# facebookresearch/PoseDiffusion

Measured on AMD Instinct MI355X. Metric: sequences/sec (20-frame, GGS on), higher is better.
Workload: dtype f32 (GGS, attention, LayerNorm, DDPM update, every accumulation); the encoder GEMMs multiply fp16 hi + lo operand pairs (22 bits, static power-of-two scales) with fp32 accumulation -- `exact_mode` is the same pipe with them on the exact-fp32 matrix instruction

## Files before the change

### posediffusion_amd/csrc/pd_denoiser.hip

```cpp
#include "pd_denoiser_dev.h"
#include "pd_gemm_stream.h"
#include "pd_gemm_split.h"
#include "pd_qkv_attn.h"
#ifndef PD_STRIP_RT3
#define PD_STRIP_RT3 1
#endif
#ifndef PD_STRIP_RT1
#define PD_STRIP_RT1 0
#endif
#ifndef PD_STRIP_RT3_FF1
#define PD_STRIP_RT3_FF1 0
#endif
#ifndef PD_STRIP_K64
#define PD_STRIP_K64 true
#endif

#include <algorithm>
#include <math.h>
#include <stdlib.h>
#include <string.h>

__global__ __launch_bounds__(256) void pd_embed_rows_kernel(const float *__restrict__ x, int n_frames, int M, float *__restrict__ out) {
    const int row = blockIdx.x * 4 + (threadIdx.x >> 6), lane = threadIdx.x & 63;
    if (row >= M) return;
    float4 *dst = (float4 *)(out + (size_t)row * KFIRST_D);
    float xv[9];
#pragma unroll
    for (int d = 0; d < 9; ++d) xv[d] = x[(size_t)row * 9 + d];
    if (lane < 45) {
        float o[4];
#pragma unroll
        for (int e = 0; e < 4; ++e) {
            const int idx = 4 * lane + e, s = idx / 90, rem = idx - s * 90, d = rem / 10, kk = rem - d * 10;
            float xd = xv[0];
#pragma unroll
            for (int q = 1; q < 9; ++q) xd = (d == q) ? xv[q] : xd;
            const float a = xd * (float)(1 << kk);
// ... 656 lines not shown
            pd_set_error("pd_engine_create: a LayerNorm weight pointer is NULL");
            return PD_ERR_INVALID_ARG;
        }
        PD_TRY(m.fold_bias(&L.qkv_b, s.in_proj_w, s.norm1_b, s.in_proj_b, 3 * DM, DM));
        PD_TRY(m.copy(&L.out_b, s.out_proj_b, DM));
        PD_TRY(m.fold_bias(&L.ff1_b, s.linear1_w, s.norm2_b, s.linear1_b, DFF, DM));
        PD_TRY(m.copy(&L.ff2_b, s.linear2_b, DM));
        PD_TRY(m.rowmajor(&L.qkv_wf, s.in_proj_w, 3 * DM, DM, s.norm1_w));
        PD_TRY(m.rowmajor(&L.out_wf, s.out_proj_w, DM, DM, nullptr));
        PD_TRY(m.rowmajor(&L.ff1_wf, s.linear1_w, DFF, DM, s.norm2_w));
        PD_TRY(m.rowmajor(&L.ff2_wf, s.linear2_w, DM, DFF, nullptr));
    }
    PD_TRY(m.copy(&d->last0_b, w->last0_b, HID));
    PD_TRY(m.copy(&d->last_ln_w, w->last_ln_w, HID));
    PD_TRY(m.copy(&d->last_ln_b, w->last_ln_b, HID));
    PD_TRY(m.copy(&d->last3_w, w->last3_w, 9 * HID));
    PD_TRY(m.copy(&d->last3_b, w->last3_b, 9));
    const size_t rows = (size_t)d->m_cap;
    PD_TRY(m.alloc(&d->h, rows * DM));
    PD_TRY(m.alloc(&d->qkv, rows * 3 * DM));
    PD_TRY(m.alloc(&d->ctx, rows * DM));
    PD_TRY(m.alloc(&d->ff, rows * DFF));
    PD_TRY(m.alloc(&d->hid, rows * HID));
    if (rows >= PD_STREAM_MIN_ROWS) PD_TRY(m.alloc(&d->hn, rows * DM));
    if (d->hn) {
        PD_TRY(m.alloc(&d->emb, rows * KFIRST_D));
        PD_TRY(m.alloc(&d->zproj, rows * DM));
        PD_TRY(m.alloc(&d->first_df, (size_t)DM * KFIRST_D));
        PD_TRY(m.alloc(&d->first_zf, (size_t)DM * ZD));
        hipLaunchKernelGGL(pd_first_rowmajor_kernel, dim3((DM * KFIRST_D + 255) / 256), dim3(256), 0, 0, w->first_w, d->first_df, PD_FIRST_D, KFIRST_D);
        hipLaunchKernelGGL(pd_first_rowmajor_kernel, dim3((DM * ZD + 255) / 256), dim3(256), 0, 0, w->first_w, d->first_zf, PD_FIRST_Z, ZD);
        PD_HIP_CHECK(hipGetLastError());
        PD_TRY(m.alloc(&d->ttab, (size_t)w->timesteps * DM));
        hipLaunchKernelGGL(pd_first_ttab_kernel, dim3(w->timesteps), dim3(DM), 0, 0, w->first_w, d->t_table, d->ttab);
        PD_HIP_CHECK(hipGetLastError());
    }
    PD_TRY(m.rowmajor(&d->last0_wf, w->last0_w, HID, DM, nullptr));
    PD_TRY(pd_set_lds(pd_gemm_kernel<KFIRST_PAD, 2, 0, 32>, 32 * (KFIRST_PAD + 4) * 4));
    PD_TRY(pd_set_lds(pd_gemm_kernel<KFIRST_PAD, 2, 0, 16>, 32 * (KFIRST_PAD + 4) * 4));
    PD_TRY(pd_set_lds(pd_gemm_kernel<DM, 1, 0, 32>, 32 * (DM + 4) * 4));
    PD_TRY(pd_set_lds(pd_gemm_kernel<DM, 1, 0, 16>, 32 * (DM + 4) * 4));
    PD_TRY(pd_set_lds(pd_gemm_kernel<DM, 1, 1, 32>, 32 * (DM + 4) * 4));
    PD_TRY(pd_set_lds(pd_gemm_kernel<DM, 1, 1, 16>, 32 * (DM + 4) * 4));
    PD_TRY(pd_set_lds(pd_gemm_kernel<DM, 0, 2, 32>, 32 * (DM + 4) * 4));
    PD_TRY(pd_set_lds(pd_gemm_kernel<DM, 0, 2, 16>, 32 * (DM + 4) * 4));
    PD_TRY(pd_set_lds(pd_gemm_kernel<DFF, 0, 2, 32>, 32 * (DFF + 4) * 4));
    PD_TRY(pd_set_lds(pd_gemm_kernel<DFF, 0, 2, 16>, 32 * (DFF + 4) * 4));
// ... 135 lines not shown
                     eng->max_B, eng->max_N, d->timesteps);
        return PD_ERR_INVALID_ARG;
    }
    if (!z_prepared) {
        int rc = pd_denoiser_prepare(eng, z, B, N, s);
        if (rc) return rc;
    }
    const int M = B * N, MT = (M + 31) / 32;
    GemmArgs g;
    memset(&g, 0, sizeof(g));
    g.M = M;
    const bool streamed = M >= PD_STREAM_MIN_ROWS && d->hn;
    if (streamed) {
        hipLaunchKernelGGL(pd_embed_rows_kernel, dim3((M + 3) / 4), dim3(256), 0, s, x, N, M, d->emb);
        pd_gemm_dma<4>(d->emb, KFIRST_D, d->first_df, KFIRST_D, d->ttab + (size_t)t * DM, d->h, M, DM, s, nullptr, d->zproj);
    } else {
        g.bias = d->first_b; g.C = d->h; g.Nout = DM;
        g.x = x; g.z = z; g.temb = d->t_table + (size_t)t * 128; g.n_frames = N;
        launch_gemm<KFIRST_PAD, 2, 0>(g, d->first_wp, MT, eng->gemm_wide_min_tiles, s);
    }
    for (int l = 0; l < d->num_layers; ++l) {
        const PdLayerDev &L = d->layers[l];
        if (streamed && eng->den_split == 2 && d->split_h_ready) {
            static const int strip = pd_dev_knob("PD_DEN_STRIP", 15);
            hipLaunchKernelGGL((pd_ln_rows_kernel<DM, 2>), dim3((M + 3) / 4), dim3(256), 0, s, d->h, d->hn, M, 1e-5f, 512.0f);
            static const int attn_mma = pd_dev_knob("PD_DEN_ATTN_MMA", 1);
            const int qa_wgs = ((B + pd_qkv_attn_group(N > 32 ? 1 : N) - 1) / pd_qkv_attn_group(N > 32 ? 1 : N)) * NH, cus = eng->num_cus > 0 ? eng->num_cus : 256;
            const bool qa_fills = 4 * qa_wgs >= 3 * ((qa_wgs + cus - 1) / cus) * cus;
            if (N <= 32 && eng->den_fused_attn == 1 ? qa_fills : (N <= 32 && eng->den_fused_attn == 2)) {
                pd_qkv_attn((const unsigned *)d->hn, L.qkv_wh, L.qkv_b, (unsigned *)d->ctx, B, N, L.qkv_cs, L.ctx_scale, s);
            } else {
                if (strip & 1) pd_gemm_strip<0, 2, true, 1, PD_STRIP_K64>((const unsigned *)d->hn, DM, L.qkv_wh, DM, L.qkv_b, d->qkv, M, 3 * DM, s, L.qkv_cs);
                else pd_gemm_split<0, 1, 2, true>((const unsigned *)d->hn, DM, L.qkv_wh, DM, L.qkv_b, d->qkv, M, 3 * DM, s, L.qkv_cs);
                if (N <= 32 && attn_mma) hipLaunchKernelGGL(pd_attn_mma_kernel<2>, dim3(B * NH), dim3(256), attn_mma_lds(N), s, d->qkv, d->ctx, N, L.ctx_scale);
                else hipLaunchKernelGGL(pd_attn_seq_kernel<2>, dim3(B * NH), dim3(256), attn_seq_lds(N), s, d->qkv, d->ctx, N, L.ctx_scale);
            }
            const bool rt3 = PD_STRIP_RT3 && (((M + 63) / 64) * (DM / 128)) > cus && (((M + 95) / 96) * (DM / 128)) <= cus;
#if PD_STRIP_RT1
            if ((strip & 2) && rt3) pd_gemm_strip<2, 1, true, 1, PD_STRIP_K64>((const unsigned *)d->ctx, DM, L.out_wh, DM, L.out_b, d->h, M, DM, s, L.out_cs);
            else
#endif
            if ((strip & 2) && rt3) pd_gemm_strip<2, 3, true, 1, PD_STRIP_K64>((const unsigned *)d->ctx, DM, L.out_wh, DM, L.out_b, d->h, M, DM, s, L.out_cs);
            else if (strip & 2) pd_gemm_strip<2, 2, true, 1, PD_STRIP_K64>((const unsigned *)d->ctx, DM, L.out_wh, DM, L.out_b, d->h, M, DM, s, L.out_cs);
            else pd_gemm_split<2, 1, 1, true>((const unsigned *)d->ctx, DM, L.out_wh, DM, L.out_b, d->h, M, DM, s, L.out_cs);
            hipLaunchKernelGGL((pd_ln_rows_kernel<DM, 2>), dim3((M + 3) / 4), dim3(256), 0, s, d->h, d->hn, M, 1e-5f, 512.0f);
#if PD_STRIP_RT1 == 2
            if ((strip & 4) && rt3) pd_gemm_strip<4, 1, true, 1, PD_STRIP_K64>((const unsigned *)d->hn, DM, L.ff1_wh, DM, L.ff1_b, d->ff, M, DFF, s, L.ff1_cs, L.ff_scale);
            else
#endif
            if ((strip & 4) && PD_STRIP_RT3_FF1 && rt3) pd_gemm_strip<4, 3, true, 1, PD_STRIP_K64>((const unsigned *)d->hn, DM, L.ff1_wh, DM, L.ff1_b, d->ff, M, DFF, s, L.ff1_cs, L.ff_scale);
            else if (strip & 4) pd_gemm_strip<4, 2, true, 1, PD_STRIP_K64>((const unsigned *)d->hn, DM, L.ff1_wh, DM, L.ff1_b, d->ff, M, DFF, s, L.ff1_cs, L.ff_scale);
            else pd_gemm_split<4, 1, 2, true>((const unsigned *)d->hn, DM, L.ff1_wh, DM, L.ff1_b, d->ff, M, DFF, s, L.ff1_cs, L.ff_scale);
#if PD_STRIP_RT1
            if ((strip & 8) && rt3) pd_gemm_strip<2, 1, true, 1, PD_STRIP_K64>((const unsigned *)d->ff, DFF, L.ff2_wh, DFF, L.ff2_b, d->h, M, DM, s, L.ff2_cs);
            else
#endif
            if ((strip & 8) && rt3) pd_gemm_strip<2, 3, true, 1, PD_STRIP_K64>((const unsigned *)d->ff, DFF, L.ff2_wh, DFF, L.ff2_b, d->h, M, DM, s, L.ff2_cs);
            else if (strip & 8) pd_gemm_strip<2, 2, true, 1, PD_STRIP_K64>((const unsigned *)d->ff, DFF, L.ff2_wh, DFF, L.ff2_b, d->h, M, DM, s, L.ff2_cs);
            else pd_gemm_split<2, 1, 1, true>((const unsigned *)d->ff, DFF, L.ff2_wh, DFF, L.ff2_b, d->h, M, DM, s, L.ff2_cs);
            continue;
        }
        if (streamed && eng->den_split == 1 && d->split_ready) {
            hipLaunchKernelGGL((pd_ln_rows_kernel<DM, 1>), dim3((M + 3) / 4), dim3(256), 0, s, d->h, d->hn, M, 1e-5f, 1.0f);
            pd_gemm_split<0, 1, 2>((const unsigned *)d->hn, DM, L.qkv_ws, DM, L.qkv_b, d->qkv, M, 3 * DM, s);
            hipLaunchKernelGGL(pd_attn_seq_kernel<1>, dim3(B * NH), dim3(256), attn_seq_lds(N), s, d->qkv, d->ctx, N, 1.0f);
            pd_gemm_split<2, 1, 1>((const unsigned *)d->ctx, DM, L.out_ws, DM, L.out_b, d->h, M, DM, s);
            hipLaunchKernelGGL((pd_ln_rows_kernel<DM, 1>), dim3((M + 3) / 4), dim3(256), 0, s, d->h, d->hn, M, 1e-5f, 1.0f);
            pd_gemm_split<4, 1, 2>((const unsigned *)d->hn, DM, L.ff1_ws, DM, L.ff1_b, d->ff, M, DFF, s);
            pd_gemm_split<2, 1, 1>((const unsigned *)d->ff, DFF, L.ff2_ws, DFF, L.ff2_b, d->h, M, DM, s);
            continue;
        }
        if (streamed) {
            float2 *stats = (float2 *)d->hn;
            hipLaunchKernelGGL(pd_ln_stats_kernel<DM>, dim3((M + 3) / 4), dim3(256), 0, s, d->h, stats, M, 1e-5f);
            pd_gemm_dma<0, true>(d->h, DM, L.qkv_wf, DM, L.qkv_b, d->qkv, M, 3 * DM, s, stats);
            hipLaunchKernelGGL(pd_attn_seq_kernel<0>, dim3(B * NH), dim3(256), attn_seq_lds(N), s, d->qkv, d->ctx, N, 1.0f);
            pd_gemm_dma<2>(d->ctx, DM, L.out_wf, DM, L.out_b, d->h, M, DM, s);
            hipLaunchKernelGGL(pd_ln_stats_kernel<DM>, dim3((M + 3) / 4), dim3(256), 0, s, d->h, stats, M, 1e-5f);
            pd_gemm_dma<1, true>(d->h, DM, L.ff1_wf, DM, L.ff1_b, d->ff, M, DFF, s, stats);
            pd_gemm_dma<2>(d->ff, DFF, L.ff2_wf, DFF, L.ff2_b, d->h, M, DM, s);
            continue;
        }
// ... 101 lines not shown
```

### posediffusion_amd/csrc/pd_denoiser_dev.h

```cpp
#pragma once
#include "pd_weight_prep.h"

#include <vector>

typedef float f32x16 __attribute__((ext_vector_type(16)));
typedef float f32x4 __attribute__((ext_vector_type(4)));

#define DM 512
#define NH 4
#define DH 128
#define DFF 1024
#define ZD 384
#define KFIRST 702
#define KFIRST_PAD 704
__host__ __device__ inline int pd_first_col_all(int kp) {
    if (kp < 384) return 317 + kp;
    if (kp < 512) return 189 + (kp - 384);
    if (kp < 692) return kp - 512;
    if (kp < 701) return 180 + (kp - 692);
    return kp;
}
#define PD_FIRST_D 1
#define PD_FIRST_Z 2
#define PD_FIRST_T 3
// ... 8 lines not shown

struct PdLayerDev {
    float *qkv_wp[2], *qkv_b;
    float *out_wp[2], *out_b;
    float *ff1_wp[2], *ff1_b;
    float *ff2_wp[2], *ff2_b;
    float *qkv_wf, *out_wf, *ff1_wf, *ff2_wf;
    unsigned *qkv_ws, *out_ws, *ff1_ws, *ff2_ws;
    unsigned *qkv_wh, *out_wh, *ff1_wh, *ff2_wh;
    float qkv_cs, out_cs, ff1_cs, ff2_cs, ctx_scale, ff_scale;
};

struct PdDenoiserDev {
    int num_layers = 0, timesteps = 0, m_cap = 0;
    float *t_table = nullptr;
    float *first_wp[2] = {nullptr, nullptr}, *first_b = nullptr;
    float *ttab = nullptr;
    float *zproj = nullptr;
    PdLayerDev layers[PD_MAX_LAYERS];
    float *last0_wp[2] = {nullptr, nullptr}, *last0_b = nullptr, *last_ln_w = nullptr, *last_ln_b = nullptr;
    float *last3_w = nullptr, *last3_b = nullptr;
    float *h = nullptr, *qkv = nullptr, *ctx = nullptr, *ff = nullptr, *hid = nullptr;
    float *hn = nullptr;
    float *emb = nullptr, *first_df = nullptr, *first_zf = nullptr, *last0_wf = nullptr;
    bool split_ready = false;
    bool split_h_ready = false;
    bool non_finite = false;
    PdDevAllocs mem{"pd_engine_create"};
};

template <int CTRL>
__device__ __forceinline__ float pd_dpp_add(float v) {
    return v + __int_as_float(__builtin_amdgcn_update_dpp(0, __float_as_int(v), CTRL, 0xf, 0xf, false));
}
__device__ __forceinline__ float pd_sum8(float v) {
    v = pd_dpp_add<0xB1>(v);
    v = pd_dpp_add<0x4E>(v);
    return pd_dpp_add<0x141>(v);
}

__device__ __forceinline__ float pd_wave_max(float v) {
#pragma unroll
    for (int off = 32; off >= 1; off >>= 1) v = fmaxf(v, __shfl_xor(v, off, 64));
    return v;
}
__device__ __forceinline__ float pd_wave_sum(float v) {
// ... 6 lines not shown
```

### posediffusion_amd/csrc/pd_gemm_split.h

```cpp
#pragma once
#include "pd_gemm_stream.h"

__device__ __forceinline__ float vit_gelu_fast(float v) {
    const float x = fabsf(v) * 0.70710678118654752f;
    const float t = __builtin_amdgcn_rcpf(fmaf(0.3275911f, x, 1.0f));
    float p = fmaf(1.061405429f, t, -1.453152027f);
    p = fmaf(p, t, 1.421413741f);
    p = fmaf(p, t, -0.284496736f);
    p = fmaf(p, t, 0.254829592f);
    const float q = 0.5f * p * t * __expf(-x * x);
    return v * (v >= 0.0f ? 1.0f - q : q);
}

struct VitSplitArgs {
    const unsigned *A, *W;
    const float *bias;
    void *C;
    int M, Nout, K, lda;
    float c_scale, out_scale;
#ifdef PD_STRIP_LEGS
    long long *legs;
#endif
};
#ifndef PD_STRIP_PIPE
#define PD_STRIP_PIPE 1
#endif
#ifndef PD_STRIP_RES_AHEAD
#define PD_STRIP_RES_AHEAD 1
#endif
#ifndef PD_STRIP_WIDE_EPI
#define PD_STRIP_WIDE_EPI 1
#endif
#ifdef PD_STRIP_LEGS
#define PD_LEG(i, v) do { if (g.legs && threadIdx.x == 0) g.legs[(size_t)blockIdx.x * 8 + (i)] = (long long)(v); } while (0)
#else
#define PD_LEG(i, v) do { } while (0)
#endif

template <int EPI, int WM, int WN, bool F16 = false, int BARE = 0>
__global__ __launch_bounds__(256) void vit_gemm_split_kernel(VitSplitArgs g) {
    constexpr int KC = PD_STREAM_KC, LR = PD_STREAM_LR, TM = 64 * WM, TN = 64 * WN, GROUP = 2048 / TM;
    static_assert(KC == 32 && WM <= 2 && WN <= 2, "staging: 4 groups of 8 per row chunk, passes of 64 rows");
// ... 138 lines not shown
            const float bias = g.bias[col];
            float res[16];
            if constexpr (EPI == 2) {
#pragma unroll
                for (int i = 0; i < 16; ++i) res[i] = ((const float *)g.C)[(size_t)min(r0 + (i & 3) + 8 * (i >> 2), g.M - 1) * g.Nout + col];
            }
#pragma unroll
            for (int i = 0; i < 16; ++i) {
                const int row = r0 + (i & 3) + 8 * (i >> 2);
                float v = F16 ? fmaf(acc[mi][ni][i], g.c_scale, bias) : acc[mi][ni][i] + bias;
                if constexpr (EPI == 3) v = vit_gelu_fast(v);
                if constexpr (EPI == 4) v = pd_relu(v);
                if constexpr (EPI == 2) v += res[i];
                if (row < g.M) {
                    if constexpr (EPI == 3 || EPI == 4)
                        ((unsigned *)g.C)[(size_t)row * g.Nout + col] = pd_split_word_as<F16 ? 2 : 1>(v, g.out_scale);
                    else
                        ((float *)g.C)[(size_t)row * g.Nout + col] = v;
                }
            }
        }
}

template <int EPI, int RT, bool F16, int CT = 1, int BARE = 0, bool K64 = false>
__global__ __launch_bounds__(256) void pd_gemm_strip_kernel(VitSplitArgs g) {
    constexpr int KC = 32, TM = 32 * RT, TN = 128 * CT, GROUP = RT == 3 ? 24 : (RT == 1 ? 32 : 2048 / TM), CHA = TM * KC;
    static_assert(RT >= 1 && RT <= 4 && (CT == 1 || CT == 2), "pieces of 8 rows, RT per wave and chunk");
    extern __shared__ __attribute__((aligned(1024))) unsigned strip_lds[];
    PD_LEG(0, wall_clock64());
    PD_LEG(2, __builtin_amdgcn_s_memtime());
    const int tid = threadIdx.x, lane = tid & 63, l31 = lane & 31, hi = lane >> 5;
    const int wave = __builtin_amdgcn_readfirstlane(tid >> 6);
    const int MT = (g.M + TM - 1) / TM, NT = g.Nout / TN;
    int mtile, ntile;
    {
        const int b = blockIdx.x, full = (MT / GROUP) * GROUP * NT;
        if (b < full) {
            const int grp = b / (NT * GROUP), r = b - grp * (NT * GROUP);
            ntile = r / GROUP;
            mtile = grp * GROUP + r % GROUP;
        } else {
            const int r = b - full, rest = MT % GROUP;
            ntile = r / rest;
            mtile = (MT / GROUP) * GROUP + r % rest;
        }
    }
    const int m0 = mtile * TM, n0 = ntile * TN;
    const int prow = lane >> 3, pslot = lane & 7;
    unsigned oa[RT];
#pragma unroll
    for (int j = 0; j < RT; ++j) {
        const int r = 8 * (RT * wave + j) + prow;
        oa[j] = (unsigned)(((size_t)min(m0 + r, g.M - 1) * g.lda + 4 * (pslot ^ ((r >> 1) & 7))) * sizeof(unsigned));
    }
    const unsigned lds_a = (unsigned)(size_t)(strip_lds + RT * wave * 256);
    auto stage = [&](int kc, int buf) {
        const float *ab = (const float *)(g.A + kc * KC);
        const unsigned da = __builtin_amdgcn_readfirstlane(lds_a + buf * CHA * 4);
#pragma unroll
        for (int j = 0; j < RT; ++j) pd_dma_piece(ab, oa[j], da + j * 1024);
    };
    const int KS = g.K / 16;
    const uint4 *wq = (const uint4 *)g.W + (size_t)(n0 / 32 + CT * wave) * KS * 128 + lane;
    uint4 cw[CT][2][2], nw[CT][2][2];
    auto mma = [](const uint4 &a, const uint4 &b, const f32x16 &c) {
        if constexpr (F16) return __builtin_amdgcn_mfma_f32_32x32x16_f16(__builtin_bit_cast(f16x8, a), __builtin_bit_cast(f16x8, b), c, 0, 0, 0);
        else return __builtin_amdgcn_mfma_f32_32x32x16_bf16(__builtin_bit_cast(bf16x8, a), __builtin_bit_cast(bf16x8, b), c, 0, 0, 0);
    };
    f32x16 acc[RT][CT];
    typedef unsigned res_v4 __attribute__((ext_vector_type(4)));
    res_v4 resid[(EPI == 2 && K64) ? RT : 1][4];
    if constexpr (K64) {
        static_assert(CT == 1 && BARE == 0, "the 64-k form exists for one column tile per wave");
        typedef unsigned wv4 __attribute__((ext_vector_type(4)));
#pragma unroll
        for (int mi = 0; mi < RT; ++mi)
#pragma unroll
            for (int i = 0; i < 16; ++i) acc[mi][0][i] = 0.0f;
// ... 89 lines not shown
                __builtin_amdgcn_sched_barrier(0);
            }
#pragma unroll
            for (int mi = 0; mi < RT; ++mi) {
                if (dma_step >= 0) dma_piece_at(dma_step * RT + mi);
                __builtin_amdgcn_sched_barrier(0);
                acc[mi][0] = mmaw(ah[mi], wh, acc[mi][0]);
                __builtin_amdgcn_sched_barrier(0);
            }
        };
#endif
        wv4 a0, a1, a2, a3, b0, b1, b2, b3;
        const int nk64 = g.K / 64;
        auto resid_load = [&]() {
            const int pr_ = lane >> 3, colb_ = n0 + wave * 32 + (lane & 7) * 4;
#pragma unroll
            for (int mi = 0; mi < RT; ++mi)
#pragma unroll
                for (int q = 0; q < 4; ++q) {
                    const float *rp_ = (const float *)g.C + (size_t)min(m0 + mi * 32 + 8 * q + pr_, g.M - 1) * g.Nout + colb_;
                    asm volatile("global_load_dwordx4 %0, %1, off" : "=&v"(resid[mi][q]) : "v"(rp_) : "memory");
                }
        };
        stage64(0, 0);
        PD_STRIP_WLOAD(a0, a1, a2, a3, 0);
        PD_STRIP_WLOAD(b0, b1, b2, b3, 1);
        PD_STRIP_WAIT(0, a0, a1, a2, a3);
        PD_STRIP_WAIT(0, b0, b1, b2, b3);
        __syncthreads();
        PD_LEG(3, __builtin_amdgcn_s_memtime());
#ifdef PD_STRIP_LEGS
        long long leg_t0 = 0, leg_wb = 0, leg_wa = 0, leg_bar = 0, leg_s0 = 0, leg_s1 = 0, leg_s2 = 0, leg_s3 = 0;
#define PD_LEG_T0() leg_t0 = __builtin_amdgcn_s_memtime()
#define PD_LEG_ACC(v) v += __builtin_amdgcn_s_memtime() - leg_t0
#else
#define PD_LEG_T0() do { } while (0)
#define PD_LEG_ACC(v) do { } while (0)
#endif
        constexpr int RESN = (PD_STRIP_RES_AHEAD && EPI == 2) ? 4 * RT : 0;
        auto chunk = [&](int c, auto mode_) {
            constexpr int MODE = decltype(mode_)::value;
            const int cn = c + 1;
            const unsigned *a = strip_lds + (c & 1) * 2 * CHA + l31 * KC;
#if PD_STRIP_PIPE
            dma_cn = cn;
            dma_nb = (c + 1) & 1;
#pragma unroll
            for (int mi = 0; mi < RT; ++mi) read_mi(0, a, 0, mi);
            wait_reads(0);
            PD_LEG_T0();
            step(0, a0, a1, true, 1, a, 1, MODE == 2 ? -1 : 0);
// ... 7 lines not shown
            block(a, a0, a1, a2, a3);
#endif
            if constexpr (MODE != 2) PD_STRIP_WLOAD(a0, a1, a2, a3, 2 * cn);
            PD_LEG_T0();
            PD_STRIP_WAITN((MODE == 2 ? RESN : 2 * RT + 4), b0, b1, b2, b3);
            PD_LEG_ACC(leg_wb);
#if PD_STRIP_PIPE
            wait_reads(0);
            PD_LEG_T0();
            step(0, b0, b1, true, 1, a + CHA, 1, -1);
            PD_LEG_ACC(leg_s2);
            wait_reads(1);
            PD_LEG_T0();
            step(1, b2, b3, false, 0, a, 0, -1);
            PD_LEG_ACC(leg_s3);
#else
            block(a + CHA, b0, b1, b2, b3);
#endif
            if constexpr (MODE != 2) {
                PD_STRIP_WLOAD(b0, b1, b2, b3, 2 * cn + 1);
                if constexpr (MODE == 1 && RESN > 0) resid_load();
                PD_LEG_T0();
                PD_STRIP_WAITN((MODE == 1 ? 4 + RESN : 4), a0, a1, a2, a3);
                PD_LEG_ACC(leg_wa);
                PD_LEG_T0();
                __syncthreads();
                PD_LEG_ACC(leg_bar);
            }
        };
        if constexpr (RESN > 0) {
            if (nk64 < 2) {
                resid_load();
                asm volatile("s_waitcnt vmcnt(0)" ::: "memory");
            }
        }
        for (int c = 0; c < nk64 - 2; ++c) chunk(c, std::integral_constant<int, 0>());
        if (nk64 >= 2) chunk(nk64 - 2, std::integral_constant<int, 1>());
        chunk(nk64 - 1, std::integral_constant<int, 2>());
        PD_STRIP_WAIT(0, b0, b1, b2, b3);
#if PD_STRIP_RES_AHEAD
        if constexpr (EPI == 2) {
#pragma unroll
            for (int mi = 0; mi < RT; ++mi) asm volatile("" : "+v"(resid[mi][0]), "+v"(resid[mi][1]), "+v"(resid[mi][2]), "+v"(resid[mi][3]));
        }
#endif
        PD_LEG(4, __builtin_amdgcn_s_memtime());
// ... 104 lines not shown
#else
                        res4[q] = *(const float4 *)((const float *)g.C + (size_t)min(m0 + mi * 32 + 8 * q + pr, g.M - 1) * g.Nout + colb);
#endif
                    }
                }
#pragma unroll
                for (int q = 0; q < 4; ++q) {
                    const int row = m0 + mi * 32 + 8 * q + pr;
                    const float4 a4 = *(const float4 *)(patch + (8 * q + pr) * 36 + pc);
                    float v[4] = {a4.x, a4.y, a4.z, a4.w};
                    const float b4[4] = {bias4.x, bias4.y, bias4.z, bias4.w};
                    const float r4[4] = {EPI == 2 ? res4[q].x : 0.0f, EPI == 2 ? res4[q].y : 0.0f, EPI == 2 ? res4[q].z : 0.0f, EPI == 2 ? res4[q].w : 0.0f};
                    unsigned o[4];
#pragma unroll
                    for (int e = 0; e < 4; ++e) {
                        float t = F16 ? fmaf(v[e], g.c_scale, b4[e]) : v[e] + b4[e];
                        if constexpr (EPI == 3) t = F16 ? 0.5f * t * (1.0f + erff(t * 0.70710678118654752f)) : vit_gelu_fast(t);
                        if constexpr (EPI == 4) t = pd_relu(t);
                        if constexpr (EPI == 2) t += r4[e];
                        if constexpr (EPI == 3 || EPI == 4) o[e] = pd_split_word_as<F16 ? 2 : 1>(t, g.out_scale);
                        else o[e] = __float_as_uint(t);
                    }
                    if (row < g.M) *(uint4 *)((unsigned *)g.C + (size_t)row * g.Nout + colb) = make_uint4(o[0], o[1], o[2], o[3]);
                }
            }
        }
    } else
#endif
#pragma unroll
    for (int c = 0; c < CT; ++c) {
        const int col = n0 + (CT * wave + c) * 32 + l31;
        const float bias = g.bias[col];
#pragma unroll
        for (int mi = 0; mi < RT; ++mi) {
            const int r0 = m0 + mi * 32 + 4 * hi;
            float res[16];
            if constexpr (EPI == 2) {
#pragma unroll
                for (int i = 0; i < 16; ++i) res[i] = ((const float *)g.C)[(size_t)min(r0 + (i & 3) + 8 * (i >> 2), g.M - 1) * g.Nout + col];
            }
#pragma unroll
            for (int i = 0; i < 16; ++i) {
                const int row = r0 + (i & 3) + 8 * (i >> 2);
                float v = F16 ? fmaf(acc[mi][c][i], g.c_scale, bias) : acc[mi][c][i] + bias;
                if constexpr (EPI == 3) v = F16 ? 0.5f * v * (1.0f + erff(v * 0.70710678118654752f)) : vit_gelu_fast(v);
                if constexpr (EPI == 4) v = pd_relu(v);
                if constexpr (EPI == 2) v += res[i];
                if (row < g.M) {
                    if constexpr (EPI == 3 || EPI == 4)
                        ((unsigned *)g.C)[(size_t)row * g.Nout + col] = pd_split_word_as<F16 ? 2 : 1>(v, g.out_scale);
                    else
                        ((float *)g.C)[(size_t)row * g.Nout + col] = v;
                }
            }
        }
    }
#ifdef PD_STRIP_LEGS
    asm volatile("s_waitcnt vmcnt(0)" ::: "memory");
    PD_LEG(5, __builtin_amdgcn_s_memtime());
#ifndef PD_STRIP_STEP_CLOCKS
    PD_LEG(1, wall_clock64());
#endif
#endif
}
template <int RT, bool K64>
static constexpr size_t pd_gemm_strip_lds() { return (size_t)(K64 ? 4 : 2) * 32 * RT * 32 * sizeof(unsigned); }
template <int EPI, int RT, bool F16, int CT = 1, bool K64 = false>
static inline void pd_gemm_strip(const unsigned *A, int lda, const unsigned *W, int K, const float *bias, void *C, int M, int Nout, hipStream_t s,
                                 float c_scale = 1.0f, float out_scale = 1.0f) {
    VitSplitArgs g{A, W, bias, C, M, Nout, K, lda, c_scale, out_scale};
    constexpr int TM = 32 * RT;
    hipLaunchKernelGGL((pd_gemm_strip_kernel<EPI, RT, F16, CT, 0, K64>), dim3(((M + TM - 1) / TM) * (Nout / (128 * CT))), dim3(256),
                       (pd_gemm_strip_lds<RT, K64>()), s, g);
}

static constexpr size_t pd_split_lds(int WM) { return (size_t)2 * 64 * WM * PD_STREAM_LR * sizeof(float); }
template <int EPI, int WM, int WN, bool F16 = false>
static inline void pd_gemm_split(const unsigned *A, int lda, const unsigned *W, int K, const float *bias, void *C, int M, int Nout, hipStream_t s,
                                 float c_scale = 1.0f, float out_scale = 1.0f) {
    VitSplitArgs g{A, W, bias, C, M, Nout, K, lda, c_scale, out_scale};
    constexpr int TM = 64 * WM, TN = 64 * WN;
    hipLaunchKernelGGL((vit_gemm_split_kernel<EPI, WM, WN, F16>), dim3(((M + TM - 1) / TM) * (Nout / TN)), dim3(256), pd_split_lds(WM), s, g);
}
```

### posediffusion_amd/csrc/pd_qkv_attn.h

```cpp
#pragma once
#include "pd_gemm_split.h"

#ifndef PD_QA_XCD_MAP
#define PD_QA_XCD_MAP 1
#endif
#define PD_QA_WAVES 12
#define PD_QA_THREADS (PD_QA_WAVES * 64)
#define PD_QA_ROWS 96
#define PD_QA_LDR (3 * DH + 4)
#define PD_QA_LS 36
#ifndef PD_QA_DEEP_DEFAULT
#define PD_QA_DEEP_DEFAULT 0
#endif

struct PdQkvAttnArgs {
    const unsigned *A;
    const unsigned *W;
    const float *bias;
    unsigned *ctx;
    int B, N, G;
    float c_scale, out_scale;
};
static inline int pd_qkv_attn_group(int N) { return N >= 1 && N <= 32 ? (PD_QA_ROWS - 1) / N : 0; }
static inline size_t pd_qkv_attn_lds(int N) {
    const int G = pd_qkv_attn_group(N);
    const size_t image = (size_t)(G * N + 1) * PD_QA_LDR * sizeof(float);
    const size_t stage = (size_t)4 * PD_QA_ROWS * 32 * sizeof(unsigned);
    return (image > stage ? image : stage) + (size_t)3 * 32 * PD_QA_LS * sizeof(float);
}

template <int BARE, bool DEEP = false>
__global__ __launch_bounds__(PD_QA_THREADS) void pd_qkv_attn_kernel(PdQkvAttnArgs g) {
    constexpr int KC = 32, RT = 3, TM = PD_QA_ROWS, CHA = TM * KC, LDR = PD_QA_LDR, LS = PD_QA_LS;
    extern __shared__ __attribute__((aligned(1024))) unsigned qa_lds[];
    const int tid = threadIdx.x, lane = tid & 63, l31 = lane & 31, hi = lane >> 5;
    const int wave = __builtin_amdgcn_readfirstlane(tid >> 6);
    int head = blockIdx.x & 3, grp = blockIdx.x >> 2;
#if PD_QA_XCD_MAP == 1
    {
// ... 1 lines not shown
        if (4 * c + 4 <= ngrp) {
            head = 2 * ((r & 7) >> 2) + (r >> 3);
            grp = 4 * c + (r & 3);
        }
    }
#elif PD_QA_XCD_MAP == 2
    {
        const int ngrp = gridDim.x >> 2, c = blockIdx.x >> 5, r = blockIdx.x & 31;
        if (8 * c + 8 <= ngrp) {
            head = r >> 3;
            grp = 8 * c + (r & 7);
        }
    }
#endif
    const int N = g.N, G = g.G, M = g.B * N;
    const int seq0 = grp * G, nseq = min(G, g.B - seq0), m0 = seq0 * N, rows = nseq * N;
    const int prow = lane >> 3, pslot = lane & 7;
    unsigned oa;
    {
        const int r = 8 * wave + prow;
        oa = (unsigned)(((size_t)min(m0 + r, M - 1) * DM + 4 * (pslot ^ ((r >> 1) & 7))) * sizeof(unsigned));
    }
    const unsigned lds_a = (unsigned)(size_t)(qa_lds + wave * 256);
    const int third = wave >> 2;
    const int ntile = third * (DM / 32) + head * (DH / 32) + (wave & 3);
    constexpr int KS = DM / 16;
    const uint4 *wq = (const uint4 *)g.W + (size_t)ntile * KS * 128 + lane;
    typedef unsigned wv4 __attribute__((ext_vector_type(4)));
    f32x16 acc[RT];
#pragma unroll
    for (int mi = 0; mi < RT; ++mi)
#pragma unroll
        for (int i = 0; i < 16; ++i) acc[mi][i] = 0.0f;
    auto mmaw = [](const uint4 &a, const wv4 &b, const f32x16 &c) {
        return __builtin_amdgcn_mfma_f32_32x32x16_f16(__builtin_bit_cast(f16x8, a), __builtin_bit_cast(f16x8, b), c, 0, 0, 0);
    };
#define PD_QA_WLOAD(w0, w1, w2, w3, b)                                                                                               \
    do {                                                                                                                             \
        const uint4 *wp_ = wq + (size_t)(b) * 256;                                                                                   \
        asm volatile("global_load_dwordx4 %0, %4, off\n\tglobal_load_dwordx4 %1, %4, off offset:1024\n\t"                           \
                     "global_load_dwordx4 %2, %4, off offset:2048\n\tglobal_load_dwordx4 %3, %4, off offset:3072"                    \
                     : "=&v"(w0), "=&v"(w1), "=&v"(w2), "=&v"(w3) : "v"(wp_) : "memory");                                            \
    } while (0)
#define PD_QA_WAIT(n, w0, w1, w2, w3) asm volatile("s_waitcnt vmcnt(" #n ")" : "+v"(w0), "+v"(w1), "+v"(w2), "+v"(w3) : : "memory")
    auto stage64 = [&](int c, int buf) {
        const unsigned da = __builtin_amdgcn_readfirstlane(lds_a + buf * 2 * CHA * 4);
// ... 5 lines not shown
#pragma unroll
        for (int st = 0; st < 2; ++st) {
#pragma unroll
            for (int mi = 0; mi < RT; ++mi) {
                const uint4 p = *(const uint4 *)(a + mi * 32 * KC + 4 * ((4 * st + 2 * hi) ^ ((l31 >> 1) & 7)));
                const uint4 q = *(const uint4 *)(a + mi * 32 * KC + 4 * ((4 * st + 2 * hi + 1) ^ ((l31 >> 1) & 7)));
                ah[mi] = make_uint4(__builtin_amdgcn_perm(p.y, p.x, 0x05040100u), __builtin_amdgcn_perm(p.w, p.z, 0x05040100u),
                                    __builtin_amdgcn_perm(q.y, q.x, 0x05040100u), __builtin_amdgcn_perm(q.w, q.z, 0x05040100u));
                al[mi] = make_uint4(__builtin_amdgcn_perm(p.y, p.x, 0x07060302u), __builtin_amdgcn_perm(p.w, p.z, 0x07060302u),
                                    __builtin_amdgcn_perm(q.y, q.x, 0x07060302u), __builtin_amdgcn_perm(q.w, q.z, 0x07060302u));
            }
            const wv4 &wh = st ? w2 : w0, &wl = st ? w3 : w1;
#pragma unroll
            for (int mi = 0; mi < RT; ++mi) acc[mi] = mmaw(al[mi], wh, acc[mi]);
#pragma unroll
            for (int mi = 0; mi < RT; ++mi) acc[mi] = mmaw(ah[mi], wl, acc[mi]);
#pragma unroll
            for (int mi = 0; mi < RT; ++mi) acc[mi] = mmaw(ah[mi], wh, acc[mi]);
        }
    };
    {
        wv4 a0, a1, a2, a3, b0, b1, b2, b3;
        constexpr int nk64 = DM / 64;
        stage64(0, 0);
        PD_QA_WLOAD(a0, a1, a2, a3, 0);
        PD_QA_WLOAD(b0, b1, b2, b3, 1);
        PD_QA_WAIT(0, a0, a1, a2, a3);
        PD_QA_WAIT(0, b0, b1, b2, b3);
        __syncthreads();
        if constexpr (DEEP) {
            static_assert(!DEEP || BARE == 0, "the deep form has no development variants");
            wv4 c0, c1, c2, c3, d0, d1, d2, d3;
            for (int c = 0; c < nk64; c += 2) {
                {
                    const unsigned *a = qa_lds + 0 * 2 * CHA + l31 * KC;
                    stage64(c + 1, 1);
                    PD_QA_WLOAD(c0, c1, c2, c3, 2 * (c + 1));
                    PD_QA_WLOAD(d0, d1, d2, d3, 2 * (c + 1) + 1);
                    block(a, a0, a1, a2, a3);
                    block(a + CHA, b0, b1, b2, b3);
                    PD_QA_WAIT(0, c0, c1, c2, c3);
                    PD_QA_WAIT(0, d0, d1, d2, d3);
                    __syncthreads();
                }
                {
                    const int cn = min(c + 2, nk64 - 1);
                    const unsigned *a = qa_lds + 1 * 2 * CHA + l31 * KC;
                    stage64(cn, 0);
                    PD_QA_WLOAD(a0, a1, a2, a3, 2 * cn);
                    PD_QA_WLOAD(b0, b1, b2, b3, 2 * cn + 1);
                    block(a, c0, c1, c2, c3);
                    block(a + CHA, d0, d1, d2, d3);
                    PD_QA_WAIT(0, a0, a1, a2, a3);
                    PD_QA_WAIT(0, b0, b1, b2, b3);
                    __syncthreads();
                }
            }
        } else
        for (int c = 0; c < nk64; ++c) {
            const int cn = min(c + 1, nk64 - 1);
            const unsigned *a = qa_lds + (c & 1) * 2 * CHA + l31 * KC;
            if constexpr (BARE == 0) {
                if (c + 1 < nk64) {
                    stage64(cn, (c + 1) & 1);
                    block(a, a0, a1, a2, a3);
                    PD_QA_WLOAD(a0, a1, a2, a3, 2 * cn);
                    PD_QA_WAIT(6, b0, b1, b2, b3);
                    block(a + CHA, b0, b1, b2, b3);
                    PD_QA_WLOAD(b0, b1, b2, b3, 2 * cn + 1);
                    PD_QA_WAIT(4, a0, a1, a2, a3);
                } else {
                    block(a, a0, a1, a2, a3);
                    PD_QA_WAIT(0, b0, b1, b2, b3);
                    block(a + CHA, b0, b1, b2, b3);
                }
            } else {
                if constexpr (BARE != 2 && BARE != 3) stage64(cn, (c + 1) & 1);
                if constexpr (BARE != 4) block(a, a0, a1, a2, a3);
                if constexpr (BARE != 1 && BARE != 3) PD_QA_WLOAD(a0, a1, a2, a3, 2 * cn);
                if constexpr (BARE != 4) block(a + CHA, b0, b1, b2, b3);
                if constexpr (BARE != 1 && BARE != 3) PD_QA_WLOAD(b0, b1, b2, b3, 2 * cn + 1);
                PD_QA_WAIT(0, a0, a1, a2, a3);
                PD_QA_WAIT(0, b0, b1, b2, b3);
            }
            __syncthreads();
        }
        PD_QA_WAIT(0, b0, b1, b2, b3);
    }
#undef PD_QA_WLOAD
#undef PD_QA_WAIT
    if constexpr (BARE == 5) {
        if (acc[0][0] == 123.456f) g.ctx[tid] = 1u;
        return;
    }
    float *img = (float *)qa_lds;
    float *Sall = img + (size_t)(G * N + 1) * LDR;
    {
        const int col = ntile * 32 + l31;
        const float bias = g.bias[col];
        const int lcol = third * DH + (wave & 3) * 32 + l31;
        const float qscale = 0.08838834764831845f;
#pragma unroll
        for (int mi = 0; mi < RT; ++mi)
#pragma unroll
            for (int i = 0; i < 16; ++i) {
                const int row = mi * 32 + 4 * hi + (i & 3) + 8 * (i >> 2);
// ... 76 lines not shown
                for (int e = 0; e < 4; ++e) {
                    o[0][0] = __builtin_amdgcn_mfma_f32_16x16x4f32(a0[e], v0[e], o[0][0], 0, 0, 0);
                    o[0][1] = __builtin_amdgcn_mfma_f32_16x16x4f32(a0[e], v1[e], o[0][1], 0, 0, 0);
                    o[1][0] = __builtin_amdgcn_mfma_f32_16x16x4f32(a1[e], v0[e], o[1][0], 0, 0, 0);
                    o[1][1] = __builtin_amdgcn_mfma_f32_16x16x4f32(a1[e], v1[e], o[1][1], 0, 0, 0);
                }
            }
#pragma unroll
            for (int rt = 0; rt < 2; ++rt)
#pragma unroll
                for (int e = 0; e < 4; ++e) {
                    const int i = 16 * rt + 4 * (lane >> 4) + e;
                    if (i < N) {
                        unsigned *out = g.ctx + (size_t)((seq0 + s) * N + i) * DM + head * DH + 32 * tw + (lane & 15);
#pragma unroll
                        for (int ct = 0; ct < 2; ++ct) out[16 * ct] = pd_split_word_as<2>(o[rt][ct][e], g.out_scale);
                    }
                }
        }
        __syncthreads();
    }
}

static inline void pd_qkv_attn(const unsigned *hn, const unsigned *Wh, const float *bias, unsigned *ctx, int B, int N, float c_scale, float out_scale,
                               hipStream_t s) {
    const int G = pd_qkv_attn_group(N);
    PdQkvAttnArgs g{hn, Wh, bias, ctx, B, N, G, c_scale, out_scale};
#ifdef PD_DEV_KNOBS
    static const int bare = pd_dev_knob("PD_QA_BARE", 0);
    const dim3 grid(((B + G - 1) / G) * NH), blk(PD_QA_THREADS);
    const size_t lds = pd_qkv_attn_lds(N);
    static const int deep = pd_dev_knob("PD_QA_DEEP", PD_QA_DEEP_DEFAULT);
    if (bare == 0 && !deep) { hipLaunchKernelGGL((pd_qkv_attn_kernel<0, false>), grid, blk, lds, s, g); return; }
    switch (bare) {
    case 1: hipLaunchKernelGGL(pd_qkv_attn_kernel<1>, grid, blk, lds, s, g); return;
    case 2: hipLaunchKernelGGL(pd_qkv_attn_kernel<2>, grid, blk, lds, s, g); return;
    case 3: hipLaunchKernelGGL(pd_qkv_attn_kernel<3>, grid, blk, lds, s, g); return;
    case 4: hipLaunchKernelGGL(pd_qkv_attn_kernel<4>, grid, blk, lds, s, g); return;
    case 5: hipLaunchKernelGGL(pd_qkv_attn_kernel<5>, grid, blk, lds, s, g); return;
    default: break;
    }
#endif
    hipLaunchKernelGGL((pd_qkv_attn_kernel<0, PD_QA_DEEP_DEFAULT != 0>), dim3(((B + G - 1) / G) * NH), dim3(PD_QA_THREADS), pd_qkv_attn_lds(N), s, g);
}
```

Measured before the change: 1139.

## Fold LayerNorm into GEMM prologues via per-slice statistics from residual epilogues

Removes the two standalone LayerNorm row kernels per layer. The residual-writing GEMM epilogues now emit per-32-column mean/M2 partials, and the consuming QKV/FF1 GEMMs (and the fused QKV-attention kernel) combine these into row statistics, then normalize and split raw fp32 h tiles in LDS before the MMA. This saves a full read/write pass of h to hn and two launches per layer, but adds conversion work and a barrier-adjacent LDS pass inside the GEMM main loops, plus a small extra partials buffer. The dev knob that allowed falling back to the split GEMM path is also dropped.

```diff
diff --git a/posediffusion_amd/csrc/pd_denoiser.hip b/posediffusion_amd/csrc/pd_denoiser.hip
--- a/posediffusion_amd/csrc/pd_denoiser.hip
+++ b/posediffusion_amd/csrc/pd_denoiser.hip
@@ -10,9 +10,6 @@
 #endif
 #ifndef PD_STRIP_RT3_FF1
 #define PD_STRIP_RT3_FF1 0
-#endif
-#ifndef PD_STRIP_K64
-#define PD_STRIP_K64 true
 #endif
 
 #include <algorithm>
@@ -715,7 +712,10 @@
     PD_TRY(m.alloc(&d->ctx, rows * DM));
     PD_TRY(m.alloc(&d->ff, rows * DFF));
     PD_TRY(m.alloc(&d->hid, rows * HID));
-    if (rows >= PD_STREAM_MIN_ROWS) PD_TRY(m.alloc(&d->hn, rows * DM));
+    if (rows >= PD_STREAM_MIN_ROWS) {
+        PD_TRY(m.alloc(&d->hn, rows * DM));
+        PD_TRY(m.alloc(&d->ln_part, rows * PD_LN_SLICES));
+    }
     if (d->hn) {
         PD_TRY(m.alloc(&d->emb, rows * KFIRST_D));
         PD_TRY(m.alloc(&d->zproj, rows * DM));
@@ -897,42 +897,40 @@
     for (int l = 0; l < d->num_layers; ++l) {
         const PdLayerDev &L = d->layers[l];
         if (streamed && eng->den_split == 2 && d->split_h_ready) {
-            static const int strip = pd_dev_knob("PD_DEN_STRIP", 15);
-            hipLaunchKernelGGL((pd_ln_rows_kernel<DM, 2>), dim3((M + 3) / 4), dim3(256), 0, s, d->h, d->hn, M, 1e-5f, 512.0f);
+            static_assert(DM == 32 * PD_LN_SLICES, "the partials cover 512-wide rows");
+            constexpr float LN_SCALE = 512.0f;
+            if (l == 0) hipLaunchKernelGGL(pd_ln_part_kernel<DM>, dim3((M + 3) / 4), dim3(256), 0, s, d->h, d->ln_part, M);
+            float2 *part_out = l + 1 < d->num_layers ? d->ln_part : nullptr;
+            const unsigned *hA = (const unsigned *)d->h;
             static const int attn_mma = pd_dev_knob("PD_DEN_ATTN_MMA", 1);
             const int qa_wgs = ((B + pd_qkv_attn_group(N > 32 ? 1 : N) - 1) / pd_qkv_attn_group(N > 32 ? 1 : N)) * NH, cus = eng->num_cus > 0 ? eng->num_cus : 256;
             const bool qa_fills = 4 * qa_wgs >= 3 * ((qa_wgs + cus - 1) / cus) * cus;
             if (N <= 32 && eng->den_fused_attn == 1 ? qa_fills : (N <= 32 && eng->den_fused_attn == 2)) {
-                pd_qkv_attn((const unsigned *)d->hn, L.qkv_wh, L.qkv_b, (unsigned *)d->ctx, B, N, L.qkv_cs, L.ctx_scale, s);
+                pd_qkv_attn(d->h, d->ln_part, LN_SCALE, L.qkv_wh, L.qkv_b, (unsigned *)d->ctx, B, N, L.qkv_cs, L.ctx_scale, s);
             } else {
-                if (strip & 1) pd_gemm_strip<0, 2, true, 1, PD_STRIP_K64>((const unsigned *)d->hn, DM, L.qkv_wh, DM, L.qkv_b, d->qkv, M, 3 * DM, s, L.qkv_cs);
-                else pd_gemm_split<0, 1, 2, true>((const unsigned *)d->hn, DM, L.qkv_wh, DM, L.qkv_b, d->qkv, M, 3 * DM, s, L.qkv_cs);
+                pd_gemm_strip<0, 2, true, 1, true, true>(hA, DM, L.qkv_wh, DM, L.qkv_b, d->qkv, M, 3 * DM, s, L.qkv_cs, 1.0f, d->ln_part, LN_SCALE);
                 if (N <= 32 && attn_mma) hipLaunchKernelGGL(pd_attn_mma_kernel<2>, dim3(B * NH), dim3(256), attn_mma_lds(N), s, d->qkv, d->ctx, N, L.ctx_scale);
                 else hipLaunchKernelGGL(pd_attn_seq_kernel<2>, dim3(B * NH), dim3(256), attn_seq_lds(N), s, d->qkv, d->ctx, N, L.ctx_scale);
             }
             const bool rt3 = PD_STRIP_RT3 && (((M + 63) / 64) * (DM / 128)) > cus && (((M + 95) / 96) * (DM / 128)) <= cus;
 #if PD_STRIP_RT1
-            if ((strip & 2) && rt3) pd_gemm_strip<2, 1, true, 1, PD_STRIP_K64>((const unsigned *)d->ctx, DM, L.out_wh, DM, L.out_b, d->h, M, DM, s, L.out_cs);
+            if (rt3) pd_gemm_strip<2, 1, true, 1, true, true>((const unsigned *)d->ctx, DM, L.out_wh, DM, L.out_b, d->h, M, DM, s, L.out_cs, 1.0f, d->ln_part);
             else
 #endif
-            if ((strip & 2) && rt3) pd_gemm_strip<2, 3, true, 1, PD_STRIP_K64>((const unsigned *)d->ctx, DM, L.out_wh, DM, L.out_b, d->h, M, DM, s, L.out_cs);
-            else if (strip & 2) pd_gemm_strip<2, 2, true, 1, PD_STRIP_K64>((const unsigned *)d->ctx, DM, L.out_wh, DM, L.out_b, d->h, M, DM, s, L.out_cs);
-            else pd_gemm_split<2, 1, 1, true>((const unsigned *)d->ctx, DM, L.out_wh, DM, L.out_b, d->h, M, DM, s, L.out_cs);
-            hipLaunchKernelGGL((pd_ln_rows_kernel<DM, 2>), dim3((M + 3) / 4), dim3(256), 0, s, d->h, d->hn, M, 1e-5f, 512.0f);
+            if (rt3) pd_gemm_strip<2, 3, true, 1, true, true>((const unsigned *)d->ctx, DM, L.out_wh, DM, L.out_b, d->h, M, DM, s, L.out_cs, 1.0f, d->ln_part);
+            else pd_gemm_strip<2, 2, true, 1, true, true>((const unsigned *)d->ctx, DM, L.out_wh, DM, L.out_b, d->h, M, DM, s, L.out_cs, 1.0f, d->ln_part);
 #if PD_STRIP_RT1 == 2
-            if ((strip & 4) && rt3) pd_gemm_strip<4, 1, true, 1, PD_STRIP_K64>((const unsigned *)d->hn, DM, L.ff1_wh, DM, L.ff1_b, d->ff, M, DFF, s, L.ff1_cs, L.ff_scale);
+            if (rt3) pd_gemm_strip<4, 1, true, 1, true, true>(hA, DM, L.ff1_wh, DM, L.ff1_b, d->ff, M, DFF, s, L.ff1_cs, L.ff_scale, d->ln_part, LN_SCALE);
             else
 #endif
-            if ((strip & 4) && PD_STRIP_RT3_FF1 && rt3) pd_gemm_strip<4, 3, true, 1, PD_STRIP_K64>((const unsigned *)d->hn, DM, L.ff1_wh, DM, L.ff1_b, d->ff, M, DFF, s, L.ff1_cs, L.ff_scale);
-            else if (strip & 4) pd_gemm_strip<4, 2, true, 1, PD_STRIP_K64>((const unsigned *)d->hn, DM, L.ff1_wh, DM, L.ff1_b, d->ff, M, DFF, s, L.ff1_cs, L.ff_scale);
-            else pd_gemm_split<4, 1, 2, true>((const unsigned *)d->hn, DM, L.ff1_wh, DM, L.ff1_b, d->ff, M, DFF, s, L.ff1_cs, L.ff_scale);
+            if (PD_STRIP_RT3_FF1 && rt3) pd_gemm_strip<4, 3, true, 1, true, true>(hA, DM, L.ff1_wh, DM, L.ff1_b, d->ff, M, DFF, s, L.ff1_cs, L.ff_scale, d->ln_part, LN_SCALE);
+            else pd_gemm_strip<4, 2, true, 1, true, true>(hA, DM, L.ff1_wh, DM, L.ff1_b, d->ff, M, DFF, s, L.ff1_cs, L.ff_scale, d->ln_part, LN_SCALE);
 #if PD_STRIP_RT1
-            if ((strip & 8) && rt3) pd_gemm_strip<2, 1, true, 1, PD_STRIP_K64>((const unsigned *)d->ff, DFF, L.ff2_wh, DFF, L.ff2_b, d->h, M, DM, s, L.ff2_cs);
+            if (rt3) pd_gemm_strip<2, 1, true, 1, true, true>((const unsigned *)d->ff, DFF, L.ff2_wh, DFF, L.ff2_b, d->h, M, DM, s, L.ff2_cs, 1.0f, part_out);
             else
 #endif
-            if ((strip & 8) && rt3) pd_gemm_strip<2, 3, true, 1, PD_STRIP_K64>((const unsigned *)d->ff, DFF, L.ff2_wh, DFF, L.ff2_b, d->h, M, DM, s, L.ff2_cs);
-            else if (strip & 8) pd_gemm_strip<2, 2, true, 1, PD_STRIP_K64>((const unsigned *)d->ff, DFF, L.ff2_wh, DFF, L.ff2_b, d->h, M, DM, s, L.ff2_cs);
-            else pd_gemm_split<2, 1, 1, true>((const unsigned *)d->ff, DFF, L.ff2_wh, DFF, L.ff2_b, d->h, M, DM, s, L.ff2_cs);
+            if (rt3) pd_gemm_strip<2, 3, true, 1, true, true>((const unsigned *)d->ff, DFF, L.ff2_wh, DFF, L.ff2_b, d->h, M, DM, s, L.ff2_cs, 1.0f, part_out);
+            else pd_gemm_strip<2, 2, true, 1, true, true>((const unsigned *)d->ff, DFF, L.ff2_wh, DFF, L.ff2_b, d->h, M, DM, s, L.ff2_cs, 1.0f, part_out);
             continue;
         }
         if (streamed && eng->den_split == 1 && d->split_ready) {
diff --git a/posediffusion_amd/csrc/pd_denoiser_dev.h b/posediffusion_amd/csrc/pd_denoiser_dev.h
--- a/posediffusion_amd/csrc/pd_denoiser_dev.h
+++ b/posediffusion_amd/csrc/pd_denoiser_dev.h
@@ -54,6 +54,7 @@
     float *last3_w = nullptr, *last3_b = nullptr;
     float *h = nullptr, *qkv = nullptr, *ctx = nullptr, *ff = nullptr, *hid = nullptr;
     float *hn = nullptr;
+    float2 *ln_part = nullptr;
     float *emb = nullptr, *first_df = nullptr, *first_zf = nullptr, *last0_wf = nullptr;
     bool split_ready = false;
     bool split_h_ready = false;
diff --git a/posediffusion_amd/csrc/pd_gemm_split.h b/posediffusion_amd/csrc/pd_gemm_split.h
--- a/posediffusion_amd/csrc/pd_gemm_split.h
+++ b/posediffusion_amd/csrc/pd_gemm_split.h
@@ -18,6 +18,8 @@
     void *C;
     int M, Nout, K, lda;
     float c_scale, out_scale;
+    float2 *ln_part;
+    float ln_scale;
 #ifdef PD_STRIP_LEGS
     long long *legs;
 #endif
@@ -202,8 +204,50 @@
         }
 }
 
-template <int EPI, int RT, bool F16, int CT = 1, int BARE = 0, bool K64 = false>
+#define PD_LN_SLICES 16
+__device__ __forceinline__ float2 pd_ln_slice(const float v[4]) {
+    const float m = pd_stream_sum8((v[0] + v[1]) + (v[2] + v[3])) * (1.0f / 32);
+    const float d0 = v[0] - m, d1 = v[1] - m, d2 = v[2] - m, d3 = v[3] - m;
+    return make_float2(m, pd_stream_sum8(fmaf(d3, d3, fmaf(d2, d2, fmaf(d1, d1, d0 * d0)))));
+}
+__device__ __forceinline__ float2 pd_ln_row_stats(const float4 &p2, float eps, float scale) {
+    const float mean = pd_stream_sum8(p2.x + p2.z) * (1.0f / PD_LN_SLICES);
+    const float da = p2.x - mean, db = p2.z - mean;
+    const float between = pd_stream_sum8(fmaf(db, db, da * da)), within = pd_stream_sum8(p2.y + p2.w);
+    const float var = fmaf(32.0f, between, within) * (1.0f / (32 * PD_LN_SLICES));
+    return make_float2(mean, scale * (1.0f / sqrtf(var + eps)));
+}
+__device__ __forceinline__ void pd_ln_convert_piece(unsigned *piece, int lane, float2 st) {
+    uint4 *p = (uint4 *)piece + lane;
+    const uint4 w = *p;
+    *p = make_uint4(pd_split_word_h((__uint_as_float(w.x) - st.x) * st.y), pd_split_word_h((__uint_as_float(w.y) - st.x) * st.y),
+                    pd_split_word_h((__uint_as_float(w.z) - st.x) * st.y), pd_split_word_h((__uint_as_float(w.w) - st.x) * st.y));
+}
+typedef unsigned pd_u32x4 __attribute__((ext_vector_type(4)));
+__device__ __forceinline__ pd_u32x4 pd_ln_part_load(const float2 *part, int row, int pslot) {
+    pd_u32x4 v;
+    const float2 *src = part + (size_t)row * PD_LN_SLICES + 2 * pslot;
+    asm volatile("global_load_dwordx4 %0, %1, off" : "=&v"(v) : "v"(src) : "memory");
+    return v;
+}
+template <int D>
+__global__ __launch_bounds__(256) void pd_ln_part_kernel(const float *__restrict__ x, float2 *__restrict__ part, int M) {
+    static_assert(D == 32 * PD_LN_SLICES, "16 slices of 32");
+    const int row = blockIdx.x * 4 + (threadIdx.x >> 6), lane = threadIdx.x & 63;
+    if (row >= M) return;
+#pragma unroll
+    for (int i = 0; i < D / 256; ++i) {
+        const float4 v4 = *((const float4 *)(x + (size_t)row * D + 256 * i) + lane);
+        const float v[4] = {v4.x, v4.y, v4.z, v4.w};
+        const float2 sl = pd_ln_slice(v);
+        if ((lane & 7) == 0) part[(size_t)row * PD_LN_SLICES + 8 * i + (lane >> 3)] = sl;
+    }
+}
+
+template <int EPI, int RT, bool F16, int CT = 1, int BARE = 0, bool K64 = false, bool LN = false>
 __global__ __launch_bounds__(256) void pd_gemm_strip_kernel(VitSplitArgs g) {
+    constexpr bool LN_A = LN && EPI != 2, LN_P = LN && EPI == 2;
+    static_assert(!LN || (K64 && F16 && CT == 1), "the LayerNorm fold exists for the 64-k fp16-plane form");
     constexpr int KC = 32, TM = 32 * RT, TN = 128 * CT, GROUP = RT == 3 ? 24 : (RT == 1 ? 32 : 2048 / TM), CHA = TM * KC;
     static_assert(RT >= 1 && RT <= 4 && (CT == 1 || CT == 2), "pieces of 8 rows, RT per wave and chunk");
     extern __shared__ __attribute__((aligned(1024))) unsigned strip_lds[];
@@ -234,6 +278,18 @@
         oa[j] = (unsigned)(((size_t)min(m0 + r, g.M - 1) * g.lda + 4 * (pslot ^ ((r >> 1) & 7))) * sizeof(unsigned));
     }
     const unsigned lds_a = (unsigned)(size_t)(strip_lds + RT * wave * 256);
+    float2 *ln_lds = (float2 *)(strip_lds + 4 * CHA);
+    pd_u32x4 ln_raw[LN_A ? RT : 1];
+    auto ln_convert = [&](int buf) {
+        if constexpr (LN_A) {
+#pragma unroll
+            for (int j = 0; j < RT; ++j) {
+                const float2 st = ln_lds[8 * (RT * wave + j) + prow];
+#pragma unroll
+                for (int h = 0; h < 2; ++h) pd_ln_convert_piece(strip_lds + buf * 2 * CHA + h * CHA + (RT * wave + j) * 256, lane, st);
+            }
+        }
+    };
     auto stage = [&](int kc, int buf) {
         const float *ab = (const float *)(g.A + kc * KC);
         const unsigned da = __builtin_amdgcn_readfirstlane(lds_a + buf * CHA * 4);
@@ -369,11 +425,24 @@
                     asm volatile("global_load_dwordx4 %0, %1, off" : "=&v"(resid[mi][q]) : "v"(rp_) : "memory");
                 }
         };
+        if constexpr (LN_A) {
+#pragma unroll
+            for (int j = 0; j < RT; ++j) ln_raw[j] = pd_ln_part_load(g.ln_part, min(m0 + 8 * (RT * wave + j) + prow, g.M - 1), pslot);
+        }
         stage64(0, 0);
         PD_STRIP_WLOAD(a0, a1, a2, a3, 0);
         PD_STRIP_WLOAD(b0, b1, b2, b3, 1);
         PD_STRIP_WAIT(0, a0, a1, a2, a3);
         PD_STRIP_WAIT(0, b0, b1, b2, b3);
+        if constexpr (LN_A) {
+#pragma unroll
+            for (int j = 0; j < RT; ++j) {
+                asm volatile("" : "+v"(ln_raw[j]));
+                const float2 st = pd_ln_row_stats(__builtin_bit_cast(float4, ln_raw[j]), 1e-5f, g.ln_scale);
+                if (pslot == 0) ln_lds[8 * (RT * wave + j) + prow] = st;
+            }
+            ln_convert(0);
+        }
         __syncthreads();
         PD_LEG(3, __builtin_amdgcn_s_memtime());
 #ifdef PD_STRIP_LEGS
@@ -427,6 +496,7 @@
                 if constexpr (MODE == 1 && RESN > 0) resid_load();
                 PD_LEG_T0();
                 PD_STRIP_WAITN((MODE == 1 ? 4 + RESN : 4), a0, a1, a2, a3);
+                ln_convert((c + 1) & 1);
                 PD_LEG_ACC(leg_wa);
                 PD_LEG_T0();
                 __syncthreads();
@@ -577,6 +647,13 @@
                         else o[e] = __float_as_uint(t);
                     }
                     if (row < g.M) *(uint4 *)((unsigned *)g.C + (size_t)row * g.Nout + colb) = make_uint4(o[0], o[1], o[2], o[3]);
+                    if constexpr (LN_P) {
+                        if (g.ln_part) {
+                            const float t4[4] = {__uint_as_float(o[0]), __uint_as_float(o[1]), __uint_as_float(o[2]), __uint_as_float(o[3])};
+                            const float2 sl = pd_ln_slice(t4);
+                            if ((lane & 7) == 0 && row < g.M) g.ln_part[(size_t)row * (g.Nout / 32) + (colb >> 5)] = sl;
+                        }
+                    }
                 }
             }
         }
@@ -618,15 +695,15 @@
 #endif
 #endif
 }
-template <int RT, bool K64>
-static constexpr size_t pd_gemm_strip_lds() { return (size_t)(K64 ? 4 : 2) * 32 * RT * 32 * sizeof(unsigned); }
-template <int EPI, int RT, bool F16, int CT = 1, bool K64 = false>
+template <int RT, bool K64, bool LN = false>
+static constexpr size_t pd_gemm_strip_lds() { return (size_t)(K64 ? 4 : 2) * 32 * RT * 32 * sizeof(unsigned) + (LN ? 32 * RT * sizeof(float2) : 0); }
+template <int EPI, int RT, bool F16, int CT = 1, bool K64 = false, bool LN = false>
 static inline void pd_gemm_strip(const unsigned *A, int lda, const unsigned *W, int K, const float *bias, void *C, int M, int Nout, hipStream_t s,
-                                 float c_scale = 1.0f, float out_scale = 1.0f) {
-    VitSplitArgs g{A, W, bias, C, M, Nout, K, lda, c_scale, out_scale};
+                                 float c_scale = 1.0f, float out_scale = 1.0f, float2 *ln_part = nullptr, float ln_scale = 1.0f) {
+    VitSplitArgs g{A, W, bias, C, M, Nout, K, lda, c_scale, out_scale, ln_part, ln_scale};
     constexpr int TM = 32 * RT;
-    hipLaunchKernelGGL((pd_gemm_strip_kernel<EPI, RT, F16, CT, 0, K64>), dim3(((M + TM - 1) / TM) * (Nout / (128 * CT))), dim3(256),
-                       (pd_gemm_strip_lds<RT, K64>()), s, g);
+    hipLaunchKernelGGL((pd_gemm_strip_kernel<EPI, RT, F16, CT, 0, K64, LN>), dim3(((M + TM - 1) / TM) * (Nout / (128 * CT))), dim3(256),
+                       (pd_gemm_strip_lds<RT, K64, LN && EPI != 2>()), s, g);
 }
 
 static constexpr size_t pd_split_lds(int WM) { return (size_t)2 * 64 * WM * PD_STREAM_LR * sizeof(float); }
diff --git a/posediffusion_amd/csrc/pd_qkv_attn.h b/posediffusion_amd/csrc/pd_qkv_attn.h
--- a/posediffusion_amd/csrc/pd_qkv_attn.h
+++ b/posediffusion_amd/csrc/pd_qkv_attn.h
@@ -15,6 +15,8 @@
 
 struct PdQkvAttnArgs {
     const unsigned *A;
+    const float2 *ln_part;
+    float ln_scale;
     const unsigned *W;
     const float *bias;
     unsigned *ctx;
@@ -62,6 +64,11 @@
         oa = (unsigned)(((size_t)min(m0 + r, M - 1) * DM + 4 * (pslot ^ ((r >> 1) & 7))) * sizeof(unsigned));
     }
     const unsigned lds_a = (unsigned)(size_t)(qa_lds + wave * 256);
+    float2 ln_st;
+    auto ln_convert = [&](int buf) {
+#pragma unroll
+        for (int h = 0; h < 2; ++h) pd_ln_convert_piece(qa_lds + buf * 2 * CHA + h * CHA + wave * 256, lane, ln_st);
+    };
     const int third = wave >> 2;
     const int ntile = third * (DM / 32) + head * (DH / 32) + (wave & 3);
     constexpr int KS = DM / 16;
@@ -113,11 +120,15 @@
     {
         wv4 a0, a1, a2, a3, b0, b1, b2, b3;
         constexpr int nk64 = DM / 64;
+        pd_u32x4 ln_raw = pd_ln_part_load(g.ln_part, min(m0 + 8 * wave + prow, M - 1), pslot);
         stage64(0, 0);
         PD_QA_WLOAD(a0, a1, a2, a3, 0);
         PD_QA_WLOAD(b0, b1, b2, b3, 1);
         PD_QA_WAIT(0, a0, a1, a2, a3);
         PD_QA_WAIT(0, b0, b1, b2, b3);
+        asm volatile("" : "+v"(ln_raw));
+        ln_st = pd_ln_row_stats(__builtin_bit_cast(float4, ln_raw), 1e-5f, g.ln_scale);
+        ln_convert(0);
         __syncthreads();
         if constexpr (DEEP) {
             static_assert(!DEEP || BARE == 0, "the deep form has no development variants");
@@ -132,6 +143,7 @@
                     block(a + CHA, b0, b1, b2, b3);
                     PD_QA_WAIT(0, c0, c1, c2, c3);
                     PD_QA_WAIT(0, d0, d1, d2, d3);
+                    ln_convert(1);
                     __syncthreads();
                 }
                 {
@@ -144,6 +156,7 @@
                     block(a + CHA, d0, d1, d2, d3);
                     PD_QA_WAIT(0, a0, a1, a2, a3);
                     PD_QA_WAIT(0, b0, b1, b2, b3);
+                    ln_convert(0);
                     __syncthreads();
                 }
             }
@@ -160,6 +173,7 @@
                     block(a + CHA, b0, b1, b2, b3);
                     PD_QA_WLOAD(b0, b1, b2, b3, 2 * cn + 1);
                     PD_QA_WAIT(4, a0, a1, a2, a3);
+                    ln_convert((c + 1) & 1);
                 } else {
                     block(a, a0, a1, a2, a3);
                     PD_QA_WAIT(0, b0, b1, b2, b3);
@@ -173,6 +187,7 @@
                 if constexpr (BARE != 1 && BARE != 3) PD_QA_WLOAD(b0, b1, b2, b3, 2 * cn + 1);
                 PD_QA_WAIT(0, a0, a1, a2, a3);
                 PD_QA_WAIT(0, b0, b1, b2, b3);
+                ln_convert((c + 1) & 1);
             }
             __syncthreads();
         }
@@ -295,10 +310,10 @@
     }
 }
 
-static inline void pd_qkv_attn(const unsigned *hn, const unsigned *Wh, const float *bias, unsigned *ctx, int B, int N, float c_scale, float out_scale,
-                               hipStream_t s) {
+static inline void pd_qkv_attn(const float *h, const float2 *ln_part, float ln_scale, const unsigned *Wh, const float *bias, unsigned *ctx, int B, int N,
+                               float c_scale, float out_scale, hipStream_t s) {
     const int G = pd_qkv_attn_group(N);
-    PdQkvAttnArgs g{hn, Wh, bias, ctx, B, N, G, c_scale, out_scale};
+    PdQkvAttnArgs g{(const unsigned *)h, ln_part, ln_scale, Wh, bias, ctx, B, N, G, c_scale, out_scale};
 #ifdef PD_DEV_KNOBS
     static const int bare = pd_dev_knob("PD_QA_BARE", 0);
     const dim3 grid(((B + G - 1) / G) * NH), blk(PD_QA_THREADS);
```

New measurement: 1140 (median of 6 runs). About the same (+0.1%).
